# withterm/term

Measured on NVIDIA B200. Metric: rows/sec scanned per suite (numeric business-rules suite, 100M rows x 8 cols per GPU), higher is better.
Workload: dtype f64

## Files before the change

term_b200/csrc/capi.cpp:

```cpp
#include <cstring>

#include "engine.hpp"
#include "hashpart.hpp"
#include "radix_sort.cuh"
#include "regex_dfa.hpp"

namespace tg {
const char* last_error_cstr();
Column* table_get_or_add(Table& t, const std::string& name, int32_t dtype);
void table_append_host(Table& t, const std::string& name, int32_t dtype, int64_t n, const void* values,
                       const int32_t* offsets, const uint8_t* validity, int64_t bit_offset);
void table_append_parquet_chunk(Table& t, const std::string& name, int32_t dtype, int32_t max_def_level, int32_t codec,
                                const uint8_t* chunk, int64_t n_bytes, int64_t num_values);
int32_t parquet_inspect_chunk(const uint8_t* chunk, int64_t n_bytes, tg_parquet_page* pages, int32_t cap);
int64_t parquet_chunk_validity(const uint8_t* chunk, int64_t n_bytes, int64_t num_values, uint8_t* out_bits);
int64_t parquet_snappy_decompress(const uint8_t* src, int64_t n, uint8_t* dst, int64_t cap);
int64_t parquet_page_decompress(int32_t codec, const uint8_t* src, int64_t n, uint8_t* dst, int64_t cap);
void table_set_column_arrow_type(Table& t, const std::string& name, const std::string& fmt);
int64_t parquet_decode_to_plain(int32_t encoding, int32_t elem_width, const uint8_t* src, int64_t n, int64_t n_values, uint8_t* dst, int64_t cap);
void table_adopt_device(Table& t, const std::string& name, int32_t dtype, int64_t n, const void* d_values,
                        const int32_t* d_offsets, const uint8_t* d_validity, int64_t n_value_bytes);
void table_append_arrow(Table& t, const void* schema_p, const void* array_p);
}

// ... 52 lines not shown
        cudaError_t ce = cudaGetDeviceCount(&n);
        if (ce != cudaSuccess || n == 0)
            throw Error(TG_ERR_CUDA, std::string("no CUDA device available (termgpu has no CPU fallback): ") +
                                         cudaGetErrorString(ce));
        if (device < 0 || device >= n) throw Error(TG_ERR_INVALID_ARG, "device index out of range");
        TG_CUDA(cudaSetDevice(device));
        auto* h = new tg_engine();
        Engine& e = h->e;
        e.device = device;
        cudaDeviceProp prop{};
        TG_CUDA(cudaGetDeviceProperties(&prop, device));
        e.sm_count = prop.multiProcessorCount;
        TG_CUDA(cudaStreamCreateWithFlags(&e.stream, cudaStreamNonBlocking));
        TG_CUDA(cudaStreamCreateWithFlags(&e.copy_stream, cudaStreamNonBlocking));
        for (auto& ev : e.ev) TG_CUDA(cudaEventCreate(&ev));
        e.pinned_bytes = 32u << 20;
        for (int i = 0; i < 2; ++i) {
            TG_CUDA(cudaMallocHost(&e.pinned[i], e.pinned_bytes));
            TG_CUDA(cudaEventCreateWithFlags(&e.pinned_free[i], cudaEventDisableTiming));
        }
        *out = h;
    });
}

void tg_engine_destroy(tg_engine* h) {
    if (!h) return;
    Engine& e = h->e;
    cudaSetDevice(e.device);
    cudaDeviceSynchronize();
    rank_session_destroy(e);
// ... 764 lines not shown
```

term_b200/csrc/engine.cu:

```cuda
#include "engine.hpp"

#include <algorithm>
#include <cmath>
#include <cstdlib>
#include <cstring>
#include <ctime>

namespace tg {

constexpr size_t PINNED_CHUNK = 32u << 20;
constexpr size_t PAD = 256;

static size_t round_up(size_t x, size_t a) { return (x + a - 1) / a * a; }

uint8_t* Engine::scratch(size_t bytes) {
    if (bytes > scratch_cap) {
        TG_CUDA(cudaStreamSynchronize(stream));
        if (d_scratch) TG_CUDA(cudaFree(d_scratch));
        scratch_cap = round_up(std::max(bytes, (size_t)1 << 20), 1 << 20);
        TG_CUDA(cudaMalloc(&d_scratch, scratch_cap));
    }
    return d_scratch;
}

// ... 128 lines not shown
    for (size_t i = 0; i < tc.size(); ++i)
        if (tc[i].col == c) {
            tc[i].need_values |= need_values;
            return (int)i;
        }
    tc.push_back(TileCol{c, need_values});
    return (int)tc.size() - 1;
}

static std::string no_field_msg(const Table& t, const std::string& col) {
    return "Schema error: No field named " + col + ". Valid fields are " + t.valid_fields() + ".";
}

__global__ void scan_states_kernel(const ScanAggOut* __restrict__ out, const ScanOpMeta* __restrict__ metas, int n_ops, DevAggRec* __restrict__ states);

static void run_scan_pass(Engine& e, Table& t, Plan& p, std::vector<ScanOp>& ops) {
    if (ops.empty()) return;
    auto P = std::make_unique<ScanParams>();
    memset(P.get(), 0, sizeof(ScanParams));
    std::vector<TileCol> tcols;
    struct OpCols {
        int c0 = -1, c1 = -1;
    };
    std::vector<OpCols> oc(ops.size());
    for (size_t i = 0; i < ops.size(); ++i) {
        ScanOp& o = ops[i];
        if (o.kind == UNIT_COUNT) oc[i].c0 = tile_col_index(tcols, o.c0, false);
        else if (o.kind == UNIT_NUM_F64 || o.kind == UNIT_NUM_I64) oc[i].c0 = tile_col_index(tcols, o.c0, true);
        else if (o.kind == UNIT_PAIR) {
            oc[i].c0 = tile_col_index(tcols, o.c0, true);
            oc[i].c1 = tile_col_index(tcols, o.c1, true);
        } else if (o.kind == UNIT_PRED || o.kind == UNIT_TERMS) {
            for (size_t k = 0; k < o.pred_cols.size(); ++k) {
                bool need_values = true;
// ... 64 lines not shown
            break;
        }
    }
    if (n_stages < 2) throw Error(TG_ERR_UNSUPPORTED, "scan pass does not fit in shared memory");

    std::vector<uint32_t> val_off(tcols.size(), 0), bit_off(tcols.size(), 0);
    stage_bytes_for(tile_rows, &val_off, &bit_off);
    P->n_rows = t.n_rows;
    P->tile_rows = tile_rows;
    P->n_tiles = (t.n_rows + tile_rows - 1) / tile_rows;
    P->n_cols = (int)tcols.size();
    P->n_stages = n_stages;
    P->stage_bytes = (uint32_t)stage_bytes;
    for (size_t i = 0; i < tcols.size(); ++i) {
        Column* c = tcols[i].col;
        ScanColDesc& d = P->tab.cols[i];
        d.values = tcols[i].need_values ? c->values.p : nullptr;
        d.validity = c->validity.p;
        d.kind = c->dtype == TG_FLOAT64 ? SC_F64 : c->dtype == TG_INT64 ? SC_I64 : c->dtype == TG_BOOL ? SC_BOOL : SC_BITS;
        if (!tcols[i].need_values) d.kind = SC_BITS;
        d.smem_val_off = val_off[i];
        d.smem_bits_off = bit_off[i];
        d.pivot = c->pivot;
        d.ipivot = c->ipivot;
        d.pivot_is_element = c->pivot_set ? 1 : 0;
    }
    int term_off = 0;
    struct UnitTmp {
        ScanUnitDesc d;
        double cost;
    };
    std::vector<UnitTmp> units;
    int code_off = 0;
    for (size_t i = 0; i < ops.size(); ++i) {
        ScanOp& o = ops[i];
        int this_code_off = code_off;
        if (o.kind == UNIT_PRED) {
            for (auto ins : o.code) {
                auto fix = [&](uint8_t kind, uint16_t& idx) {
                    if (kind == PK_COL_F64 || kind == PK_COL_I64 || kind == PK_COL_I64_AS_F64 || kind == PK_COL_BOOL)
                        idx = (uint16_t)tile_col_index(tcols, o.pred_cols[idx], true);
                };
                fix(ins.a_kind, ins.a_idx);
                fix(ins.b_kind, ins.b_idx);
                P->tab.code[code_off++] = ins;
            }
        }
        if (o.kind == UNIT_TERMS) {
            this_code_off = term_off;
            for (auto tm : o.terms) {
                tm.col = tile_col_index(tcols, o.pred_cols[tm.col], false);
                if (term_off >= SCAN_MAX_TERMS) throw Error(TG_ERR_UNSUPPORTED, "too many predicate terms in one scan pass");
                P->tab.terms[term_off++] = tm;
            }
        }
        const int r = reps[i];
        const int chunks = tile_rows / 128;
        for (int k = 0; k < r; ++k) {
            UnitTmp u{};
            u.d.kind = o.kind;
            u.d.c0 = oc[i].c0;
            u.d.c1 = oc[i].c1;
            u.d.row0 = (k * chunks / r) * 128;
            u.d.nrows = ((k + 1) * chunks / r) * 128 - u.d.row0;
            u.d.agg = (int)i;
            u.d.code_off = this_code_off;
            u.d.code_len = o.kind == UNIT_TERMS ? (int)o.terms.size() : (int)o.code.size();
            u.d.c0_is_i64 = o.c0 && o.c0->dtype == TG_INT64;
// ... 3 lines not shown
            units.push_back(u);
        }
    }
    std::vector<int> order(units.size());
    for (size_t i = 0; i < order.size(); ++i) order[i] = (int)i;
    std::stable_sort(order.begin(), order.end(), [&](int a, int b) { return units[a].cost > units[b].cost; });
    double load[SCAN_CONSUMER_WARPS] = {0};
    int owned[SCAN_CONSUMER_WARPS] = {0};
    for (int idx : order) {
        int best = -1;
        for (int w = 0; w < SCAN_CONSUMER_WARPS; ++w)
            if (owned[w] < SCAN_WARP_UNITS && (best < 0 || load[w] < load[best])) best = w;
        if (best < 0) throw Error(TG_ERR_UNSUPPORTED, "too many aggregates in one scan pass");
        units[idx].d.warp = best;
        load[best] += units[idx].cost;
        P->tab.warp_units[best][1 + owned[best]] = idx;
        P->tab.warp_units[best][0] = ++owned[best];
    }
    P->n_units = (int)units.size();
    P->n_state_units = units.size() <= (size_t)SCAN_CONSUMER_WARPS ? 0 : (int)units.size();
    P->n_aggs = (int)ops.size();
    P->n_code = code_off;
    P->n_terms = term_off;
    for (size_t i = 0; i < units.size(); ++i) P->tab.units[i] = units[i].d;

    const int grid = (int)std::min<int64_t>(std::max<int64_t>(P->n_tiles, 1), e.sm_count);
    const size_t partial_bytes = (size_t)grid * P->n_units * SCAN_STATE_SLOTS * 8;
    const size_t out_bytes = ops.size() * sizeof(ScanAggOut);
    uint8_t* scr = e.scratch(round_up(partial_bytes, 256) + out_bytes);
    P->partials = reinterpret_cast<uint64_t*>(scr);
    ScanAggOut* d_out = reinterpret_cast<ScanAggOut*>(scr + round_up(partial_bytes, 256));

    TG_CUDA(cudaEventRecord(e.ev[0], e.stream));
    TG_CUDA(scan_launch(*P, grid, d_out, e.stream));
    TG_CUDA(cudaEventRecord(e.ev[1], e.stream));
    e.launches += 2;
    p.stats.launches += 2;
    if (e.fused) {
        FusedScan& fz = *e.fused;
        ScanOpMeta* hm = fz.h_metas + fz.n_metas;
        for (size_t i = 0; i < ops.size(); ++i) {
            hm[i] = ScanOpMeta{ops[i].kind, ops[i].agg, ops[i].c0 ? ops[i].c0->pivot : 0.0, ops[i].c1 ? ops[i].c1->pivot : 0.0, (uint64_t)t.n_rows};
            fz.from_device[ops[i].agg] = 1;
        }
        scan_states_kernel<<<1, 64, 0, e.stream>>>(d_out, hm, (int)ops.size(), fz.d_states);
        TG_CUDA(cudaGetLastError());
        fz.n_metas += (int)ops.size();
        e.launches += 1;
        p.stats.launches += 1;
        return;
    }
    ScanAggOut* h_out = reinterpret_cast<ScanAggOut*>(e.host_scratch(out_bytes));
    TG_CUDA(cudaMemcpyAsync(h_out, d_out, out_bytes, cudaMemcpyDeviceToHost, e.stream));
    TG_CUDA(cudaStreamSynchronize(e.stream));
    float ms = 0;
    TG_CUDA(cudaEventElapsedTime(&ms, e.ev[0], e.ev[1]));
    p.stats.scan_ms += ms;
    p.stats.gpu_ms += ms;

    auto u2d = [](uint64_t u) {
        double d;
        memcpy(&d, &u, 8);
        return d;
    };
    for (size_t i = 0; i < ops.size(); ++i) {
        Agg& a = p.aggs[ops[i].agg];
        const uint64_t* s = h_out[i].s;
        switch (ops[i].kind) {
            case UNIT_COUNT:
                a.u[0] = (uint64_t)t.n_rows;
                a.u[1] = s[S_N];
                break;
            case UNIT_NUM_F64:
            case UNIT_NUM_I64:
                a.u[0] = s[S_N];
                a.f[0] = ops[i].c0->pivot;
                a.f[1] = u2d(s[S_SD]);
                a.f[2] = u2d(s[S_SDD]);
                a.f[5] = (double)s[S_N] * ops[i].c0->pivot + u2d(s[S_SD]);
                if (ops[i].kind == UNIT_NUM_I64) {
                    a.u[1] = s[S_ISUM];
                    a.u[2] = s[S_MIN];
                    a.u[3] = s[S_MAX];
                    a.u[4] = 1;
                } else {
                    a.f[3] = u2d(s[S_MIN]);
                    a.f[4] = u2d(s[S_MAX]);
                }
                break;
            case UNIT_PAIR:
                a.u[0] = s[P_N];
                a.f[0] = ops[i].c0->pivot;
                a.f[1] = ops[i].c1->pivot;
                a.f[2] = u2d(s[P_SX]);
                a.f[3] = u2d(s[P_SY]);
                a.f[4] = u2d(s[P_SXX]);
                a.f[5] = u2d(s[P_SYY]);
                a.f[6] = u2d(s[P_SXY]);
                break;
            case UNIT_PRED:
            case UNIT_TERMS:
                a.u[0] = s[0];
                a.u[1] = ops[i].kind == UNIT_PRED ? s[1] : 0;
                a.u[2] = (uint64_t)t.n_rows;
                break;
        }
    }
}
// ... 89 lines not shown

__global__ void widen_kernel(const uint32_t* __restrict__ src, uint64_t* __restrict__ dst, int64_t n, int is_float) {
    for (int64_t i = (int64_t)blockIdx.x * blockDim.x + threadIdx.x; i < n; i += (int64_t)gridDim.x * blockDim.x) {
        const uint32_t v = __ldg(src + i);
        dst[i] = is_float ? (uint64_t)__double_as_longlong((double)__uint_as_float(v)) : (uint64_t)(int64_t)(int32_t)v;
    }
}

Column* numeric_view(Engine& e, Column* c) {
    if (!c) return nullptr;
    if (c->dtype == TG_INT64 || c->dtype == TG_FLOAT64) return c;
    if (c->dtype != TG_INT32 && c->dtype != TG_FLOAT32) return nullptr;
    if (!c->wide) c->wide = std::make_unique<Column>();
    Column& w = *c->wide;
    if (w.n_rows != c->n_rows || !w.values.p) {
        e.sync_copies();
        w.name = c->name;
        w.dtype = c->dtype == TG_INT32 ? TG_INT64 : TG_FLOAT64;
        e.dev_reserve(w.values, (size_t)c->n_rows * 8, 0);
        if (c->n_rows > 0) {
            const int grid = (int)std::max<int64_t>(1, std::min<int64_t>((c->n_rows + 255) / 256, (int64_t)e.sm_count * 16));
            widen_kernel<<<grid, 256, 0, e.stream>>>(reinterpret_cast<const uint32_t*>(c->values.p), reinterpret_cast<uint64_t*>(w.values.p),
                                                     c->n_rows, c->dtype == TG_FLOAT32 ? 1 : 0);
            TG_CUDA(cudaGetLastError());
            e.launches += 1;
            const int64_t head = std::min<int64_t>(c->n_rows, 65536);
            std::vector<uint8_t> hv((size_t)head * 8), hb((size_t)(head + 7) / 8);
            TG_CUDA(cudaMemcpyAsync(hv.data(), w.values.p, hv.size(), cudaMemcpyDeviceToHost, e.stream));
            if (c->validity.p) TG_CUDA(cudaMemcpyAsync(hb.data(), c->validity.p, hb.size(), cudaMemcpyDeviceToHost, e.stream));
            TG_CUDA(cudaStreamSynchronize(e.stream));
// ... 510 lines not shown
            }
            if (t.n_rows > 0) {
                str_like_kernel<<<grid, 256, 0, e.stream>>>((const int32_t*)col->offsets.p, col->values.p, t.n_rows, d_tok, d_tok + m, (int32_t)m,
                                                            (uint32_t*)v->values.p);
                launched();
            }
            p.stats.bytes_scanned += (uint64_t)(t.n_rows + 1) * 4 + (uint64_t)col->value_bytes;
            return col_node(v);
        }
    }
    auto copy = std::make_shared<Expr>(*ex);
    for (auto& a : copy->args) a = rewrite_string_compares(a, e, t, p, vc);
    return copy;
}

void exec_scan_jobs(Engine& e, Table& t, Plan& p, const std::vector<int>& agg_ids) {
    VirtualCols virtuals(e);
    std::vector<ScanOp> ops;
    uint64_t bytes = 0;
    std::vector<Column*> counted_vals, counted_bits;
    auto count_bytes = [&](Column* c, bool values) {
        if (values && std::find(counted_vals.begin(), counted_vals.end(), c) == counted_vals.end()) {
            counted_vals.push_back(c);
            bytes += c->dtype == TG_BOOL ? (uint64_t)(t.n_rows + 7) / 8 : (uint64_t)t.n_rows * 8;
        }
        if (c->validity.p && std::find(counted_bits.begin(), counted_bits.end(), c) == counted_bits.end()) {
            counted_bits.push_back(c);
            bytes += (uint64_t)(t.n_rows + 7) / 8;
        }
    };
    std::vector<std::pair<int, int>> valid_from_num;
// ... 16 lines not shown
        ScanOp o;
        o.agg = id;
        auto col = [&](const std::string& name) -> Column* {
            Column* c = t.find(name);
            if (!c) {
                a.err = TG_ERR_COLUMN_NOT_FOUND;
                a.err_msg = no_field_msg(t, name);
            }
            return c;
        };
        auto numeric = [&](Column*& c) {
            if (Column* v = c->temporal ? nullptr : numeric_view(e, c)) {
                if (v != c || c->src_type) {
                    a.narrow = 1 | (c->src_unsigned ? 2 : 0);
                    a.narrow_name = c->src_type ? c->src_type : (c->dtype == TG_INT32 ? "Int32" : "Float32");
                }
                c = v;
                return true;
            }
            a.err = TG_ERR_TYPE_MISMATCH;
            a.err_msg = "Error during planning: numeric aggregate is not supported for column '" + c->name +
                        "' of this type";
            return false;
        };
        switch (a.kind) {
            case A_VALID: {
                Column* c = col(a.cols[0]);
                if (!c) break;
                if (!c->validity.p) {
                    a.u[0] = (uint64_t)t.n_rows;
                    a.u[1] = (uint64_t)t.n_rows;
                    break;
                }
                o.kind = UNIT_COUNT;
                o.c0 = c;
                o.cost = 0.2;
                count_bytes(c, false);
                ops.push_back(std::move(o));
            } break;
            case A_NUM: {
                Column* c = col(a.cols[0]);
                if (!c || !numeric(c)) break;
                o.kind = c->dtype == TG_INT64 ? UNIT_NUM_I64 : UNIT_NUM_F64;
                o.c0 = c;
                o.flags = a.flags ? a.flags : 7;
                if (c->dtype != TG_INT64) o.flags &= ~4;
// ... 41 lines not shown
                        compile_predicate(expr, res, o.code);
                        o.kind = UNIT_PRED;
                        o.cost = 10.0 + 25.0 * (double)o.code.size();
                    }
                } catch (Error& er) {
                    a.err = er.code;
                    a.err_msg = er.msg;
                    break;
                }
                for (auto* c : o.pred_cols) count_bytes(c, true);
                ops.push_back(std::move(o));
            } break;
            default: break;
        }
    }
    p.stats.bytes_scanned += bytes;
    struct FoldFill {
        Plan& p;
        Table& t;
        std::vector<std::pair<int, int>>& v;
        ~FoldFill() {
            if (p_fused) {
                for (auto& pr : v) p_fused->folds.push_back(pr);
                return;
            }
            for (auto& pr : v) {
                p.aggs[pr.first].u[0] = (uint64_t)t.n_rows;
                p.aggs[pr.first].u[1] = p.aggs[pr.second].u[0];
            }
        }
        FusedScan* p_fused;
    } fold_fill{p, t, valid_from_num, e.fused};
    if (t.n_rows == 0) {
        for (auto& o : ops)
            if (p.aggs[o.agg].kind == A_PRED) p.aggs[o.agg].u[2] = 0;
        return;
    }
    auto ordinal = [&](const ScanOp& o) {
        const Column* c = o.c0 ? o.c0 : (o.pred_cols.empty() ? nullptr : o.pred_cols[0]);
        if (!c) return -1;
        for (size_t i = 0; i < t.cols.size(); ++i)
            if (t.cols[i].get() == c || t.cols[i]->wide.get() == c) return (int)i;
        return (int)t.cols.size();
    };
    std::vector<std::pair<int, size_t>> op_key(ops.size());
    for (size_t i = 0; i < ops.size(); ++i) op_key[i] = {ordinal(ops[i]), i};
    std::stable_sort(op_key.begin(), op_key.end(), [](const std::pair<int, size_t>& a, const std::pair<int, size_t>& b) { return a.first < b.first; });
    {
// ... 15 lines not shown
        std::vector<ScanOp> pass;
        int code = 0, terms = 0;
        std::vector<const Column*> cols;
        while (i < ops.size() && pass.size() < (size_t)SCAN_CONSUMER_WARPS) {
            const int add_code = (int)ops[i].code.size();
            const int add_terms = ops[i].kind == UNIT_TERMS ? (int)ops[i].terms.size() : 0;
            std::vector<const Column*> with = cols;
            op_cols(ops[i], with);
            if (!pass.empty() && (code + add_code > SCAN_MAX_CODE || terms + add_terms > SCAN_MAX_TERMS || with.size() > (size_t)SCAN_MAX_COLS)) break;
            code += add_code;
            terms += add_terms;
            cols.swap(with);
            pass.push_back(std::move(ops[i]));
            ++i;
        }
        std::vector<int> pass_aggs;
        for (auto& o : pass) pass_aggs.push_back(o.agg);
        try {
            run_scan_pass(e, t, p, pass);
        } catch (Error& er) {
            if (er.code == TG_ERR_CUDA) throw;
            for (int id : pass_aggs) {
                p.aggs[id].err = er.code;
                p.aggs[id].err_msg = er.msg;
            }
        }
    }
}


void execute_partial(Engine& e, Plan& p, const std::string& table_name) {
    std::lock_guard<std::mutex> g(e.mu);
    TG_CUDA(cudaSetDevice(e.device));
    p.reset_partials();
    p.stats = tg_exec_stats{};
    p.executed = false;
    e.sync_copies();
    auto it = e.tables.find(table_name);
    Table* t = it == e.tables.end() ? nullptr : it->second.get();
    std::vector<int> scan_ids, string_ids, kll_ids, length_ids, grouped_ids;
    for (size_t i = 0; i < p.aggs.size(); ++i) {
        Agg& a = p.aggs[i];
        if (a.err != TG_OK) continue;
// ... 173 lines not shown
```

term_b200/csrc/engine.hpp:

```cpp
#pragma once
#include <cuda_runtime.h>

#include <map>
#include <memory>
#include <mutex>
#include <string>
#include <vector>

#include "common.hpp"
#include "plan.hpp"
#include "scan_defs.h"

namespace tg {

#define TG_CUDA(expr)                                                                                   \
    do {                                                                                                \
        cudaError_t _e = (expr);                                                                        \
        if (_e != cudaSuccess)                                                                          \
            throw ::tg::Error(TG_ERR_CUDA, std::string(#expr) + ": " + cudaGetErrorString(_e));         \
    } while (0)

struct Engine;
struct RankSession;

// ... 21 lines not shown
    bool adopted = false;
    std::unique_ptr<Column> wide;
    const char* src_type = nullptr;
    bool src_unsigned = false;
    bool temporal = false;
    char temporal_unit = 0;
    int elem_bytes() const {
        switch (dtype) {
            case TG_INT64: case TG_FLOAT64: return 8;
            case TG_INT32: case TG_FLOAT32: return 4;
            default: return 0;
        }
    }
};

struct Table {
    Engine* eng = nullptr;
    std::string name;
    std::vector<std::unique_ptr<Column>> cols;
    int64_t n_rows = 0;
    Column* find(const std::string& n) {
        for (auto& c : cols)
            if (c->name == n) return c.get();
        return nullptr;
    }
    std::string valid_fields() const {
        std::string s;
        for (size_t i = 0; i < cols.size(); ++i) {
            if (i) s += ", ";
            s += name + "." + cols[i]->name;
        }
        return s;
    }
};

// ... 122 lines not shown

void mailbox_create(Engine& e, int world, int rank, size_t slot_bytes, void* handle_out );
void mailbox_open(Engine& e, const void* handles );
void mailbox_destroy(Engine& e);
bool mailbox_exchange(Engine& e, const uint8_t* blob, size_t n, std::vector<std::vector<uint8_t>>& out);
void mailbox_exchange_device(Engine& e, size_t payload_bytes, std::vector<std::vector<uint8_t>>& out);

void comm_unique_id(void* id128);
void comm_init(Engine& e, const void* id128, int world, int rank);
void comm_destroy(Engine& e);
int64_t comm_shuffle_column(Engine& e, const std::string& table, const std::string& column, const std::string& shard_name, bool allow_range);
bool comm_rank_exchange(Engine& e, int64_t* n_recv, uint64_t* rank_base, uint64_t* total);
int64_t comm_shuffle_fingerprints(Engine& e, const std::string& table, const std::vector<std::string>& columns, const std::string& shard_name);

size_t scan_smem_bytes(const ScanParams& P);
cudaError_t scan_launch(const ScanParams& P, int grid, ScanAggOut* d_out, cudaStream_t stream);

}
```

term_b200/csrc/scan.cu:

```cuda
#include <cfloat>
#include <cstddef>
#include <cstdio>
#include <math_constants.h>

#include "ptx.cuh"
#include "scan_defs.h"

namespace tg {

extern __shared__ __align__(128) uint8_t scan_smem[];

typedef uint64_t Slots[SCAN_STATE_SLOTS];

__device__ __forceinline__ uint32_t tail_mask(int base_row, int rows_in_tile) {
    const int rem = rows_in_tile - base_row;
    return rem >= 32 ? 0xffffffffu : (rem <= 0 ? 0u : ((1u << rem) - 1u));
}
__device__ __forceinline__ double u2d(uint64_t u) { return __longlong_as_double((long long)u); }
__device__ __forceinline__ uint64_t d2u(double d) { return (uint64_t)__double_as_longlong(d); }

__device__ __forceinline__ uint32_t vword(const ScanColDesc& c, const uint8_t* stage, int word) {
    return c.validity ? reinterpret_cast<const uint32_t*>(stage + c.smem_bits_off)[word] : 0xffffffffu;
}
__device__ __forceinline__ uint32_t word_or_ones(const uint32_t* bits, bool has_bits, int g) { return has_bits ? bits[g] : 0xffffffffu; }
// ... 801 lines not shown
            break;
        case UNIT_TERMS: run_unit<SINGLE, TermsUnit>(p, T, ud, st, lane, stage, rows, partial); break;
        default: run_unit<SINGLE, PredUnit>(p, T, ud, st, lane, stage, rows, partial); break;
    }
}

__global__ void __launch_bounds__(SCAN_THREADS, 1) scan_kernel(const __grid_constant__ ScanParams P) {
    const int warp = threadIdx.x >> 5, lane = threadIdx.x & 31;
    uint8_t* stages = scan_smem;
    uint64_t* state = reinterpret_cast<uint64_t*>(scan_smem + (size_t)P.n_stages * P.stage_bytes);
    uint64_t* full = state + (size_t)P.n_state_units * SCAN_STATE_SLOTS * 32;
    uint64_t* empty = full + P.n_stages;
    ScanTables* T = reinterpret_cast<ScanTables*>(empty + P.n_stages);

    {
        const uint32_t* src = reinterpret_cast<const uint32_t*>(&P.tab);
        uint32_t* dst = reinterpret_cast<uint32_t*>(T);
        auto copy = [&](size_t off, size_t bytes) {
            for (uint32_t i = threadIdx.x; i < bytes / 4; i += blockDim.x) dst[off / 4 + i] = src[off / 4 + i];
        };
        copy(offsetof(ScanTables, cols), sizeof(ScanColDesc) * P.n_cols);
        copy(offsetof(ScanTables, units), sizeof(ScanUnitDesc) * P.n_units);
        copy(offsetof(ScanTables, code), sizeof(PredInstr) * P.n_code);
        copy(offsetof(ScanTables, terms), sizeof(ScanTerm) * P.n_terms);
        copy(offsetof(ScanTables, warp_units), sizeof(T->warp_units));
    }
    if (threadIdx.x == 0) {
        for (int s = 0; s < P.n_stages; ++s) {
            mbar_init(&full[s], 1);
            mbar_init(&empty[s], SCAN_CONSUMER_WARPS);
        }
// ... 81 lines not shown
            }
            __syncwarp();
            for (int k = 0; k < n_mine; ++k) {
                const int u = T->warp_units[cw][1 + k];
                const uint64_t* st = state + (size_t)u * SCAN_STATE_SLOTS * 32;
                Slots r;
#pragma unroll
                for (int sl = 0; sl < SCAN_STATE_SLOTS; ++sl) r[sl] = st[sl * 32 + lane];
                reduce_store(T->units[u].kind, r, P.partials + ((size_t)blockIdx.x * P.n_units + u) * SCAN_STATE_SLOTS, lane);
            }
        }
    }
}

constexpr int FIN_THREADS = 128;
__global__ void __launch_bounds__(FIN_THREADS) scan_finalize_kernel(const __grid_constant__ ScanParams P, int n_ctas, ScanAggOut* out) {
    const int agg = blockIdx.x, tid = threadIdx.x, lane = tid & 31, warp = tid >> 5;
    __shared__ int ulist[SCAN_MAX_UNITS];
    __shared__ int s_nu, s_kind;
    __shared__ uint64_t red[FIN_THREADS / 32][SCAN_STATE_SLOTS];
    if (tid == 0) {
        int nu = 0, kind = -1;
        for (int u = 0; u < P.n_units; ++u)
            if (P.tab.units[u].agg == agg) {
                ulist[nu++] = u;
                kind = P.tab.units[u].kind;
            }
        s_nu = nu;
        s_kind = kind;
    }
    __syncthreads();
    const int nu = s_nu, kind = s_kind;
    if (kind < 0) return;
    uint64_t acc[SCAN_STATE_SLOTS];
    int op[SCAN_STATE_SLOTS];
#pragma unroll
    for (int k = 0; k < SCAN_STATE_SLOTS; ++k) {
        op[k] = slot_op(kind, k);
        acc[k] = slot_identity(kind, k);
    }
    const int total = n_ctas * nu;
    for (int i = tid; i < total; i += FIN_THREADS) {
        const int b = i / nu, u = ulist[i - b * nu];
        const ulonglong2* rec = reinterpret_cast<const ulonglong2*>(P.partials + ((size_t)b * P.n_units + u) * SCAN_STATE_SLOTS);
#pragma unroll
        for (int k = 0; k < SCAN_STATE_SLOTS / 2; ++k) {
            const ulonglong2 v = rec[k];
            acc[2 * k] = slot_combine(op[2 * k], acc[2 * k], v.x);
            acc[2 * k + 1] = slot_combine(op[2 * k + 1], acc[2 * k + 1], v.y);
        }
    }
#pragma unroll
    for (int k = 0; k < SCAN_STATE_SLOTS; ++k) {
#pragma unroll
        for (int m = 16; m > 0; m >>= 1) acc[k] = slot_combine(op[k], acc[k], shfl_xor_u64(acc[k], m));
        if (lane == 0) red[warp][k] = acc[k];
    }
    __syncthreads();
    if (tid < SCAN_STATE_SLOTS) {
        uint64_t v = red[0][tid];
        const int o = slot_op(kind, tid);
        for (int w = 1; w < FIN_THREADS / 32; ++w) v = slot_combine(o, v, red[w][tid]);
        out[agg].s[tid] = v;
    }
}

size_t scan_smem_bytes(const ScanParams& P) {
    return (size_t)P.n_stages * P.stage_bytes + (size_t)P.n_state_units * SCAN_STATE_SLOTS * 32 * 8 +
           (size_t)2 * P.n_stages * 8 + sizeof(ScanTables);
}

cudaError_t scan_launch(const ScanParams& P, int grid, ScanAggOut* d_out, cudaStream_t stream) {
    size_t smem = scan_smem_bytes(P);
    cudaError_t e = cudaFuncSetAttribute(scan_kernel, cudaFuncAttributeMaxDynamicSharedMemorySize, 227 * 1024);
    if (e != cudaSuccess) return e;
    scan_kernel<<<grid, SCAN_THREADS, smem, stream>>>(P);
    e = cudaGetLastError();
    if (e != cudaSuccess) return e;
    scan_finalize_kernel<<<P.n_aggs, FIN_THREADS, 0, stream>>>(P, grid, d_out);
    return cudaGetLastError();
}

}
```

term_b200/csrc/scan_defs.h:

```cpp
#pragma once
#include <stdint.h>

namespace tg {

constexpr int SCAN_MAX_COLS = 32;
constexpr int SCAN_MAX_UNITS = 48;
constexpr int SCAN_MAX_CODE = 128;
constexpr int SCAN_MAX_TERMS = 32;
constexpr int SCAN_UNIT_TERMS = 4;
#ifndef TG_SCAN_CONSUMER_WARPS
#define TG_SCAN_CONSUMER_WARPS 16
#endif
constexpr int SCAN_CONSUMER_WARPS = TG_SCAN_CONSUMER_WARPS;
constexpr int SCAN_THREADS = (SCAN_CONSUMER_WARPS + 1) * 32;
constexpr int SCAN_STATE_SLOTS = 8;
constexpr int SCAN_MAX_STAGES = 8;
constexpr int SCAN_WARP_UNITS = 7;

enum : int32_t { SC_F64 = 0, SC_I64 = 1, SC_BITS = 2 , SC_BOOL = 3  };

struct ScanColDesc {
    const uint8_t* values;
    const uint8_t* validity;
    int32_t kind;
// ... 82 lines not shown
    int32_t col;
    int32_t kind;
    int32_t cmp_mask;
    int32_t pad;
    uint64_t imm;
};

struct ScanTables {
    ScanColDesc cols[SCAN_MAX_COLS];
    ScanUnitDesc units[SCAN_MAX_UNITS];
    PredInstr code[SCAN_MAX_CODE];
    ScanTerm terms[SCAN_MAX_TERMS];
    int32_t warp_units[SCAN_CONSUMER_WARPS][SCAN_WARP_UNITS + 1];
};

struct ScanParams {
    int64_t n_rows;
    int64_t n_tiles;
    int32_t tile_rows;
    int32_t n_cols;
    int32_t n_units;
    int32_t n_stages;
    uint32_t stage_bytes;
    int32_t n_aggs;
    int32_t n_code;
    int32_t n_terms;
    int32_t n_state_units;
    uint64_t* partials;
    ScanTables tab;
};

struct ScanAggOut {
    uint64_t s[SCAN_STATE_SLOTS];
};

}
```

term_b200/csrc/tables.cu:

```cuda
#include <algorithm>
#include <cstring>

#include "engine.hpp"

namespace tg {

static size_t round_up(size_t x, size_t a) { return (x + a - 1) / a * a; }

void set_pivot_host(Column& c, int32_t dtype, int64_t n, const void* values, const uint8_t* validity,
                    int64_t bit_offset) {
    if (c.pivot_set || (dtype != TG_INT64 && dtype != TG_FLOAT64)) return;
    double cand[5];
    int64_t icand[5];
    int m = 0;
    for (int64_t i = 0; i < n && i < 65536 && m < 5; ++i) {
        bool ok = !validity || ((validity[(bit_offset + i) >> 3] >> ((bit_offset + i) & 7)) & 1);
        if (!ok) continue;
        if (dtype == TG_INT64) {
            icand[m] = reinterpret_cast<const int64_t*>(values)[i];
            cand[m] = (double)icand[m];
            ++m;
        } else {
            double v = reinterpret_cast<const double*>(values)[i];
            if (v == v && v - v == 0.0) {
// ... 37 lines not shown
    } else {
        for (int64_t i = 0; i < n; ++i) {
            const int64_t s = src_off + i;
            const int bit = (src[s >> 3] >> (s & 7)) & 1;
            const int64_t o = shift + i;
            tmp[o >> 3] |= (uint8_t)(bit << (o & 7));
            z += !bit;
        }
    }
    if (zeros) *zeros = z;
    tail = (total & 7) ? tmp[out_bytes - 1] : 0;
    e.h2d(buf.p + first_byte, tmp.data(), out_bytes);
}

Column* table_get_or_add(Table& t, const std::string& name, int32_t dtype) {
    Column* c = t.find(name);
    if (c) {
        if (c->dtype != dtype) throw Error(TG_ERR_TYPE_MISMATCH, "column '" + name + "' was registered with a different type");
        return c;
    }
    validate_identifier(name);
    auto nc = std::make_unique<Column>();
    nc->name = name;
    nc->dtype = dtype;
    t.cols.push_back(std::move(nc));
    return t.cols.back().get();
}

void append_validity(Engine& e, Column& c, int64_t have, const uint8_t* validity, int64_t bit_offset, int64_t n) {
    bool has_nulls = false;
// ... 174 lines not shown
        f.dtype = TG_INT64, f.temporal = true, f.src_type = "Timestamp", f.temporal_unit = fmt[2];
    else if (fmt == "tDs" || fmt == "tDm" || fmt == "tDu" || fmt == "tDn") f.dtype = TG_INT64, f.temporal = true, f.src_type = "Duration";
    else throw Error(TG_ERR_UNSUPPORTED, std::string("Arrow format '") + fmt + "' of column '" + column + "' is not supported");
    return f;
}

void table_set_column_arrow_type(Table& t, const std::string& name, const std::string& fmt) {
    Engine& e = *t.eng;
    std::lock_guard<std::mutex> g(e.mu);
    Column* c = t.find(name);
    if (!c) throw Error(TG_ERR_COLUMN_NOT_FOUND, "Schema error: No field named " + name + ". Valid fields are " + t.valid_fields() + ".");
    const ArrowFormat f = arrow_format(fmt, name.c_str());
    if (f.dtype != c->dtype || f.large_offsets) throw Error(TG_ERR_TYPE_MISMATCH, "column '" + name + "' does not store Arrow format '" + fmt + "'");
    if (f.src_w == 4 || f.src_w == 8)
        throw Error(TG_ERR_UNSUPPORTED, "column '" + name + "': Arrow format '" + fmt + "' cannot be declared on stored values");
    c->src_type = f.src_type;
    c->src_unsigned = f.src_unsigned;
    c->temporal = f.temporal;
    c->temporal_unit = f.temporal_unit;
}

void table_append_arrow(Table& t, const void* schema_p, const void* array_p) {
    const ArrowSchema* sc = (const ArrowSchema*)schema_p;
    const ArrowArray* ar = (const ArrowArray*)array_p;
    if (!sc || !ar || !sc->format || strcmp(sc->format, "+s") != 0)
        throw Error(TG_ERR_INVALID_ARG, "expected a struct-typed ArrowArray (a RecordBatch)");
    if (ar->offset != 0) throw Error(TG_ERR_UNSUPPORTED, "sliced struct arrays are not supported");
    for (int64_t i = 0; i < sc->n_children; ++i) {
        const ArrowSchema* cs = sc->children[i];
        const ArrowArray* ca = ar->children[i];
// ... 72 lines not shown
```

Measured before the change: 191.5 billion.

## Cache compiled scan passes per table and move scan tables to device memory

Compiles each scan pass once into a cached entry keyed by aggregate definitions and env knobs. Per-pass tables, including a new precomputed finalize unit list, are uploaded once to a persistent device block, so the large ScanTables struct no longer travels as a kernel parameter. The smem opt-in attribute is set once at engine creation, and the finalize kernel batches its partial loads. The cache adds invalidation complexity: it must be cleared when columns change, and a stale entry would give wrong results.

New measurement: 195.2 billion, median of 6. 2.0% higher.

```diff
diff --git a/term_b200/csrc/capi.cpp b/term_b200/csrc/capi.cpp
--- a/term_b200/csrc/capi.cpp
+++ b/term_b200/csrc/capi.cpp
@@ -90,6 +90,7 @@
         TG_CUDA(cudaStreamCreateWithFlags(&e.stream, cudaStreamNonBlocking));
         TG_CUDA(cudaStreamCreateWithFlags(&e.copy_stream, cudaStreamNonBlocking));
         for (auto& ev : e.ev) TG_CUDA(cudaEventCreate(&ev));
+        TG_CUDA(scan_opt_in());
         e.pinned_bytes = 32u << 20;
         for (int i = 0; i < 2; ++i) {
             TG_CUDA(cudaMallocHost(&e.pinned[i], e.pinned_bytes));
diff --git a/term_b200/csrc/engine.cu b/term_b200/csrc/engine.cu
--- a/term_b200/csrc/engine.cu
+++ b/term_b200/csrc/engine.cu
@@ -166,10 +166,12 @@
 
 __global__ void scan_states_kernel(const ScanAggOut* __restrict__ out, const ScanOpMeta* __restrict__ metas, int n_ops, DevAggRec* __restrict__ states);
 
-static void run_scan_pass(Engine& e, Table& t, Plan& p, std::vector<ScanOp>& ops) {
-    if (ops.empty()) return;
-    auto P = std::make_unique<ScanParams>();
-    memset(P.get(), 0, sizeof(ScanParams));
+static CompiledPass compile_scan_pass(Engine& e, Table& t, std::vector<ScanOp>& ops) {
+    CompiledPass cp;
+    cp.host = std::make_unique<ScanPassTables>();
+    memset(cp.host.get(), 0, sizeof(ScanPassTables));
+    ScanParams* P = &cp.P;
+    ScanTables& tab = cp.host->tab;
     std::vector<TileCol> tcols;
     struct OpCols {
         int c0 = -1, c1 = -1;
@@ -264,7 +266,7 @@
     P->stage_bytes = (uint32_t)stage_bytes;
     for (size_t i = 0; i < tcols.size(); ++i) {
         Column* c = tcols[i].col;
-        ScanColDesc& d = P->tab.cols[i];
+        ScanColDesc& d = tab.cols[i];
         d.values = tcols[i].need_values ? c->values.p : nullptr;
         d.validity = c->validity.p;
         d.kind = c->dtype == TG_FLOAT64 ? SC_F64 : c->dtype == TG_INT64 ? SC_I64 : c->dtype == TG_BOOL ? SC_BOOL : SC_BITS;
@@ -293,7 +295,7 @@
                 };
                 fix(ins.a_kind, ins.a_idx);
                 fix(ins.b_kind, ins.b_idx);
-                P->tab.code[code_off++] = ins;
+                tab.code[code_off++] = ins;
             }
         }
         if (o.kind == UNIT_TERMS) {
@@ -301,7 +303,7 @@
             for (auto tm : o.terms) {
                 tm.col = tile_col_index(tcols, o.pred_cols[tm.col], false);
                 if (term_off >= SCAN_MAX_TERMS) throw Error(TG_ERR_UNSUPPORTED, "too many predicate terms in one scan pass");
-                P->tab.terms[term_off++] = tm;
+                tab.terms[term_off++] = tm;
             }
         }
         const int r = reps[i];
@@ -335,25 +337,45 @@
         if (best < 0) throw Error(TG_ERR_UNSUPPORTED, "too many aggregates in one scan pass");
         units[idx].d.warp = best;
         load[best] += units[idx].cost;
-        P->tab.warp_units[best][1 + owned[best]] = idx;
-        P->tab.warp_units[best][0] = ++owned[best];
+        tab.warp_units[best][1 + owned[best]] = idx;
+        tab.warp_units[best][0] = ++owned[best];
     }
     P->n_units = (int)units.size();
     P->n_state_units = units.size() <= (size_t)SCAN_CONSUMER_WARPS ? 0 : (int)units.size();
     P->n_aggs = (int)ops.size();
     P->n_code = code_off;
     P->n_terms = term_off;
-    for (size_t i = 0; i < units.size(); ++i) P->tab.units[i] = units[i].d;
-
-    const int grid = (int)std::min<int64_t>(std::max<int64_t>(P->n_tiles, 1), e.sm_count);
-    const size_t partial_bytes = (size_t)grid * P->n_units * SCAN_STATE_SLOTS * 8;
-    const size_t out_bytes = ops.size() * sizeof(ScanAggOut);
-    uint8_t* scr = e.scratch(round_up(partial_bytes, 256) + out_bytes);
-    P->partials = reinterpret_cast<uint64_t*>(scr);
-    ScanAggOut* d_out = reinterpret_cast<ScanAggOut*>(scr + round_up(partial_bytes, 256));
-
+    for (size_t i = 0; i < units.size(); ++i) tab.units[i] = units[i].d;
+    ScanFinalize& fin = cp.host->fin;
+    for (size_t a = 0; a < ops.size(); ++a) {
+        fin.off[a + 1] = fin.off[a];
+        for (size_t u = 0; u < units.size(); ++u)
+            if (units[u].d.agg == (int)a) {
+                fin.units[fin.off[a + 1]++] = (int)u;
+                fin.kind[a] = units[u].d.kind;
+            }
+    }
+    cp.grid = (int)std::min<int64_t>(std::max<int64_t>(P->n_tiles, 1), e.sm_count);
+    for (auto& o : ops) cp.ops.push_back(ScanPassOp{o.kind, o.agg, o.c0 ? o.c0->pivot : 0.0, o.c1 ? o.c1->pivot : 0.0});
+    return cp;
+}
+
+static size_t pass_device_bytes(const CompiledPass& cp) {
+    return round_up(cp.partial_bytes(), 256) + round_up(cp.ops.size() * sizeof(ScanAggOut), 256) + round_up(sizeof(ScanPassTables), 256);
+}
+static void place_pass(Engine& e, CompiledPass& cp, uint8_t* d) {
+    cp.P.partials = reinterpret_cast<uint64_t*>(d);
+    d += round_up(cp.partial_bytes(), 256);
+    cp.d_out = reinterpret_cast<ScanAggOut*>(d);
+    d += round_up(cp.ops.size() * sizeof(ScanAggOut), 256);
+    cp.P.tables = reinterpret_cast<const ScanPassTables*>(d);
+    TG_CUDA(cudaMemcpyAsync(d, cp.host.get(), sizeof(ScanPassTables), cudaMemcpyHostToDevice, e.stream));
+}
+
+static void run_scan_pass(Engine& e, Table& t, Plan& p, const CompiledPass& cp) {
+    const std::vector<ScanPassOp>& ops = cp.ops;
     TG_CUDA(cudaEventRecord(e.ev[0], e.stream));
-    TG_CUDA(scan_launch(*P, grid, d_out, e.stream));
+    TG_CUDA(scan_launch(cp.P, cp.grid, cp.d_out, e.stream));
     TG_CUDA(cudaEventRecord(e.ev[1], e.stream));
     e.launches += 2;
     p.stats.launches += 2;
@@ -361,18 +383,18 @@
         FusedScan& fz = *e.fused;
         ScanOpMeta* hm = fz.h_metas + fz.n_metas;
         for (size_t i = 0; i < ops.size(); ++i) {
-            hm[i] = ScanOpMeta{ops[i].kind, ops[i].agg, ops[i].c0 ? ops[i].c0->pivot : 0.0, ops[i].c1 ? ops[i].c1->pivot : 0.0, (uint64_t)t.n_rows};
+            hm[i] = ScanOpMeta{ops[i].kind, ops[i].agg, ops[i].pivot0, ops[i].pivot1, (uint64_t)t.n_rows};
             fz.from_device[ops[i].agg] = 1;
         }
-        scan_states_kernel<<<1, 64, 0, e.stream>>>(d_out, hm, (int)ops.size(), fz.d_states);
+        scan_states_kernel<<<1, 64, 0, e.stream>>>(cp.d_out, hm, (int)ops.size(), fz.d_states);
         TG_CUDA(cudaGetLastError());
         fz.n_metas += (int)ops.size();
         e.launches += 1;
         p.stats.launches += 1;
         return;
     }
-    ScanAggOut* h_out = reinterpret_cast<ScanAggOut*>(e.host_scratch(out_bytes));
-    TG_CUDA(cudaMemcpyAsync(h_out, d_out, out_bytes, cudaMemcpyDeviceToHost, e.stream));
+    const ScanAggOut* h_out = cp.h_out;
+    TG_CUDA(cudaMemcpyAsync(cp.h_out, cp.d_out, ops.size() * sizeof(ScanAggOut), cudaMemcpyDeviceToHost, e.stream));
     TG_CUDA(cudaStreamSynchronize(e.stream));
     float ms = 0;
     TG_CUDA(cudaEventElapsedTime(&ms, e.ev[0], e.ev[1]));
@@ -395,10 +417,10 @@
             case UNIT_NUM_F64:
             case UNIT_NUM_I64:
                 a.u[0] = s[S_N];
-                a.f[0] = ops[i].c0->pivot;
+                a.f[0] = ops[i].pivot0;
                 a.f[1] = u2d(s[S_SD]);
                 a.f[2] = u2d(s[S_SDD]);
-                a.f[5] = (double)s[S_N] * ops[i].c0->pivot + u2d(s[S_SD]);
+                a.f[5] = (double)s[S_N] * ops[i].pivot0 + u2d(s[S_SD]);
                 if (ops[i].kind == UNIT_NUM_I64) {
                     a.u[1] = s[S_ISUM];
                     a.u[2] = s[S_MIN];
@@ -411,8 +433,8 @@
                 break;
             case UNIT_PAIR:
                 a.u[0] = s[P_N];
-                a.f[0] = ops[i].c0->pivot;
-                a.f[1] = ops[i].c1->pivot;
+                a.f[0] = ops[i].pivot0;
+                a.f[1] = ops[i].pivot1;
                 a.f[2] = u2d(s[P_SX]);
                 a.f[3] = u2d(s[P_SY]);
                 a.f[4] = u2d(s[P_SXX]);
@@ -532,6 +554,9 @@
     if (!c->wide) c->wide = std::make_unique<Column>();
     Column& w = *c->wide;
     if (w.n_rows != c->n_rows || !w.values.p) {
+        for (auto& kv : e.tables)
+            for (auto& tc : kv.second->cols)
+                if (tc.get() == c) kv.second->clear_scan_cache();
         e.sync_copies();
         w.name = c->name;
         w.dtype = c->dtype == TG_INT32 ? TG_INT64 : TG_FLOAT64;
@@ -1072,7 +1097,59 @@
     return copy;
 }
 
+ScanCacheEntry::~ScanCacheEntry() {
+    if (d_block) eng->dev_free(d_block, d_bytes);
+    if (h_block) cudaFreeHost(h_block);
+}
+
+constexpr size_t SCAN_CACHE_ENTRIES = 8;
+
+static std::string scan_cache_key(const Plan& p, const std::vector<int>& agg_ids) {
+    std::string k;
+    for (const char* knob : {"TG_SCAN_TILE_ROWS", "TG_SCAN_MIN_STAGES", "TG_SCAN_UNITS"}) {
+        const char* v = getenv(knob);
+        k += v ? v : "";
+        k += '\x1e';
+    }
+    for (int id : agg_ids) {
+        const Agg& a = p.aggs[id];
+        k += std::to_string(id) + '\x1f' + std::to_string((int)a.kind) + '\x1f' + std::to_string(a.flags) + '\x1f' + a.key + '\x1e';
+    }
+    return k;
+}
+
+static void run_cached_scan(Engine& e, Table& t, Plan& p, const ScanCacheEntry& ce) {
+    p.stats.bytes_scanned += ce.bytes_scanned;
+    for (size_t i = 0; i < ce.narrow.size(); ++i) {
+        p.aggs[ce.narrow[i].first].narrow = ce.narrow[i].second;
+        p.aggs[ce.narrow[i].first].narrow_name = ce.narrow_name[i];
+    }
+    for (int id : ce.all_rows) {
+        p.aggs[id].u[0] = (uint64_t)t.n_rows;
+        p.aggs[id].u[1] = (uint64_t)t.n_rows;
+    }
+    for (const CompiledPass& cp : ce.passes) run_scan_pass(e, t, p, cp);
+    for (auto& pr : ce.folds) {
+        if (e.fused) {
+            e.fused->folds.push_back(pr);
+        } else {
+            p.aggs[pr.first].u[0] = (uint64_t)t.n_rows;
+            p.aggs[pr.first].u[1] = p.aggs[pr.second].u[0];
+        }
+    }
+}
+
 void exec_scan_jobs(Engine& e, Table& t, Plan& p, const std::vector<int>& agg_ids) {
+    const std::string key = scan_cache_key(p, agg_ids);
+    for (size_t i = 0; i < t.scan_cache.size(); ++i)
+        if (t.scan_cache[i]->key == key) {
+            std::rotate(t.scan_cache.begin() + i, t.scan_cache.begin() + i + 1, t.scan_cache.end());
+            run_cached_scan(e, t, p, *t.scan_cache.back());
+            return;
+        }
+    auto ce = std::make_unique<ScanCacheEntry>();
+    ce->eng = &e;
+    ce->key = key;
     VirtualCols virtuals(e);
     std::vector<ScanOp> ops;
     uint64_t bytes = 0;
@@ -1119,6 +1196,8 @@
                 if (v != c || c->src_type) {
                     a.narrow = 1 | (c->src_unsigned ? 2 : 0);
                     a.narrow_name = c->src_type ? c->src_type : (c->dtype == TG_INT32 ? "Int32" : "Float32");
+                    ce->narrow.emplace_back(id, a.narrow);
+                    ce->narrow_name.push_back(a.narrow_name);
                 }
                 c = v;
                 return true;
@@ -1133,8 +1212,7 @@
                 Column* c = col(a.cols[0]);
                 if (!c) break;
                 if (!c->validity.p) {
-                    a.u[0] = (uint64_t)t.n_rows;
-                    a.u[1] = (uint64_t)t.n_rows;
+                    ce->all_rows.push_back(id);
                     break;
                 }
                 o.kind = UNIT_COUNT;
@@ -1206,7 +1284,6 @@
             default: break;
         }
     }
-    p.stats.bytes_scanned += bytes;
     struct FoldFill {
         Plan& p;
         Table& t;
@@ -1223,7 +1300,12 @@
         }
         FusedScan* p_fused;
     } fold_fill{p, t, valid_from_num, e.fused};
+    for (int id : ce->all_rows) {
+        p.aggs[id].u[0] = (uint64_t)t.n_rows;
+        p.aggs[id].u[1] = (uint64_t)t.n_rows;
+    }
     if (t.n_rows == 0) {
+        p.stats.bytes_scanned += bytes;
         for (auto& o : ops)
             if (p.aggs[o.agg].kind == A_PRED) p.aggs[o.agg].u[2] = 0;
         return;
@@ -1269,19 +1351,54 @@
             pass.push_back(std::move(ops[i]));
             ++i;
         }
-        std::vector<int> pass_aggs;
-        for (auto& o : pass) pass_aggs.push_back(o.agg);
         try {
-            run_scan_pass(e, t, p, pass);
+            ce->passes.push_back(compile_scan_pass(e, t, pass));
         } catch (Error& er) {
             if (er.code == TG_ERR_CUDA) throw;
-            for (int id : pass_aggs) {
-                p.aggs[id].err = er.code;
-                p.aggs[id].err_msg = er.msg;
-            }
-        }
-    }
-}
+            for (auto& o : pass) {
+                p.aggs[o.agg].err = er.code;
+                p.aggs[o.agg].err_msg = er.msg;
+            }
+        }
+    }
+    bool cacheable = virtuals.cols.empty();
+    for (int id : agg_ids) cacheable &= p.aggs[id].err == TG_OK;
+    if (!cacheable) {
+        p.stats.bytes_scanned += bytes;
+        for (CompiledPass& cp : ce->passes) {
+            const size_t out_bytes = cp.ops.size() * sizeof(ScanAggOut);
+            place_pass(e, cp, e.scratch(pass_device_bytes(cp)));
+            cp.h_out = reinterpret_cast<ScanAggOut*>(e.host_scratch(out_bytes));
+            run_scan_pass(e, t, p, cp);
+        }
+        return;
+    }
+    ce->folds = valid_from_num;
+    ce->bytes_scanned = bytes;
+    fold_fill.v.clear();
+    size_t d_bytes = 0, h_bytes = 0;
+    for (const CompiledPass& cp : ce->passes) {
+        d_bytes += pass_device_bytes(cp);
+        h_bytes += round_up(cp.ops.size() * sizeof(ScanAggOut), 64);
+    }
+    if (d_bytes) {
+        ce->d_block = e.dev_alloc(d_bytes);
+        ce->d_bytes = d_bytes;
+        TG_CUDA(cudaMallocHost(&ce->h_block, h_bytes));
+    }
+    uint8_t* d = ce->d_block;
+    uint8_t* h = ce->h_block;
+    for (CompiledPass& cp : ce->passes) {
+        place_pass(e, cp, d);
+        cp.h_out = reinterpret_cast<ScanAggOut*>(h);
+        d += pass_device_bytes(cp);
+        h += round_up(cp.ops.size() * sizeof(ScanAggOut), 64);
+    }
+    if (t.scan_cache.size() >= SCAN_CACHE_ENTRIES) t.scan_cache.erase(t.scan_cache.begin());
+    t.scan_cache.push_back(std::move(ce));
+    run_cached_scan(e, t, p, *t.scan_cache.back());
+}
+
 
 
 void execute_partial(Engine& e, Plan& p, const std::string& table_name) {
diff --git a/term_b200/csrc/engine.hpp b/term_b200/csrc/engine.hpp
--- a/term_b200/csrc/engine.hpp
+++ b/term_b200/csrc/engine.hpp
@@ -59,11 +59,42 @@
     }
 };
 
+struct ScanPassOp {
+    int32_t kind, agg;
+    double pivot0, pivot1;
+};
+struct CompiledPass {
+    ScanParams P{};
+    int grid = 0;
+    std::unique_ptr<ScanPassTables> host;
+    std::vector<ScanPassOp> ops;
+    ScanAggOut* d_out = nullptr;
+    ScanAggOut* h_out = nullptr;
+    size_t partial_bytes() const { return (size_t)grid * P.n_units * SCAN_STATE_SLOTS * 8; }
+};
+
+struct ScanCacheEntry {
+    Engine* eng = nullptr;
+    std::string key;
+    std::vector<CompiledPass> passes;
+    uint64_t bytes_scanned = 0;
+    std::vector<int> all_rows;
+    std::vector<std::pair<int, int>> folds;
+    std::vector<std::pair<int, int32_t>> narrow;
+    std::vector<const char*> narrow_name;
+    uint8_t* d_block = nullptr;
+    size_t d_bytes = 0;
+    uint8_t* h_block = nullptr;
+    ~ScanCacheEntry();
+};
+
 struct Table {
     Engine* eng = nullptr;
     std::string name;
     std::vector<std::unique_ptr<Column>> cols;
     int64_t n_rows = 0;
+    std::vector<std::unique_ptr<ScanCacheEntry>> scan_cache;
+    void clear_scan_cache() { scan_cache.clear(); }
     Column* find(const std::string& n) {
         for (auto& c : cols)
             if (c->name == n) return c.get();
@@ -216,6 +247,7 @@
 int64_t comm_shuffle_fingerprints(Engine& e, const std::string& table, const std::vector<std::string>& columns, const std::string& shard_name);
 
 size_t scan_smem_bytes(const ScanParams& P);
+cudaError_t scan_opt_in();
 cudaError_t scan_launch(const ScanParams& P, int grid, ScanAggOut* d_out, cudaStream_t stream);
 
 }
diff --git a/term_b200/csrc/scan.cu b/term_b200/csrc/scan.cu
--- a/term_b200/csrc/scan.cu
+++ b/term_b200/csrc/scan.cu
@@ -839,7 +839,7 @@
     ScanTables* T = reinterpret_cast<ScanTables*>(empty + P.n_stages);
 
     {
-        const uint32_t* src = reinterpret_cast<const uint32_t*>(&P.tab);
+        const uint32_t* src = reinterpret_cast<const uint32_t*>(&P.tables->tab);
         uint32_t* dst = reinterpret_cast<uint32_t*>(T);
         auto copy = [&](size_t off, size_t bytes) {
             for (uint32_t i = threadIdx.x; i < bytes / 4; i += blockDim.x) dst[off / 4 + i] = src[off / 4 + i];
@@ -951,24 +951,15 @@
 }
 
 constexpr int FIN_THREADS = 128;
-__global__ void __launch_bounds__(FIN_THREADS) scan_finalize_kernel(const __grid_constant__ ScanParams P, int n_ctas, ScanAggOut* out) {
+__global__ void __launch_bounds__(FIN_THREADS) scan_finalize_kernel(const ScanParams P, int n_ctas, ScanAggOut* out) {
     const int agg = blockIdx.x, tid = threadIdx.x, lane = tid & 31, warp = tid >> 5;
     __shared__ int ulist[SCAN_MAX_UNITS];
-    __shared__ int s_nu, s_kind;
     __shared__ uint64_t red[FIN_THREADS / 32][SCAN_STATE_SLOTS];
-    if (tid == 0) {
-        int nu = 0, kind = -1;
-        for (int u = 0; u < P.n_units; ++u)
-            if (P.tab.units[u].agg == agg) {
-                ulist[nu++] = u;
-                kind = P.tab.units[u].kind;
-            }
-        s_nu = nu;
-        s_kind = kind;
-    }
+    const ScanFinalize& F = P.tables->fin;
+    const int u0 = F.off[agg], nu = F.off[agg + 1] - u0, kind = F.kind[agg];
+    if (tid < nu) ulist[tid] = F.units[u0 + tid];
     __syncthreads();
-    const int nu = s_nu, kind = s_kind;
-    if (kind < 0) return;
+    if (nu == 0) return;
     uint64_t acc[SCAN_STATE_SLOTS];
     int op[SCAN_STATE_SLOTS];
 #pragma unroll
@@ -977,14 +968,27 @@
         acc[k] = slot_identity(kind, k);
     }
     const int total = n_ctas * nu;
-    for (int i = tid; i < total; i += FIN_THREADS) {
-        const int b = i / nu, u = ulist[i - b * nu];
-        const ulonglong2* rec = reinterpret_cast<const ulonglong2*>(P.partials + ((size_t)b * P.n_units + u) * SCAN_STATE_SLOTS);
-#pragma unroll
-        for (int k = 0; k < SCAN_STATE_SLOTS / 2; ++k) {
-            const ulonglong2 v = rec[k];
-            acc[2 * k] = slot_combine(op[2 * k], acc[2 * k], v.x);
-            acc[2 * k + 1] = slot_combine(op[2 * k + 1], acc[2 * k + 1], v.y);
+    constexpr int FIN_BATCH = 8;
+    for (int i0 = tid; i0 < total; i0 += FIN_THREADS * FIN_BATCH) {
+        ulonglong2 v[FIN_BATCH][SCAN_STATE_SLOTS / 2];
+#pragma unroll
+        for (int j = 0; j < FIN_BATCH; ++j) {
+            const int i = i0 + j * FIN_THREADS;
+            if (i < total) {
+                const int b = i / nu, u = ulist[i - b * nu];
+                const ulonglong2* rec = reinterpret_cast<const ulonglong2*>(P.partials + ((size_t)b * P.n_units + u) * SCAN_STATE_SLOTS);
+#pragma unroll
+                for (int k = 0; k < SCAN_STATE_SLOTS / 2; ++k) v[j][k] = rec[k];
+            }
+        }
+#pragma unroll
+        for (int j = 0; j < FIN_BATCH; ++j) {
+            if (i0 + j * FIN_THREADS >= total) break;
+#pragma unroll
+            for (int k = 0; k < SCAN_STATE_SLOTS / 2; ++k) {
+                acc[2 * k] = slot_combine(op[2 * k], acc[2 * k], v[j][k].x);
+                acc[2 * k + 1] = slot_combine(op[2 * k + 1], acc[2 * k + 1], v[j][k].y);
+            }
         }
     }
 #pragma unroll
@@ -1007,12 +1011,13 @@
            (size_t)2 * P.n_stages * 8 + sizeof(ScanTables);
 }
 
+cudaError_t scan_opt_in() {
+    return cudaFuncSetAttribute(scan_kernel, cudaFuncAttributeMaxDynamicSharedMemorySize, 227 * 1024);
+}
+
 cudaError_t scan_launch(const ScanParams& P, int grid, ScanAggOut* d_out, cudaStream_t stream) {
-    size_t smem = scan_smem_bytes(P);
-    cudaError_t e = cudaFuncSetAttribute(scan_kernel, cudaFuncAttributeMaxDynamicSharedMemorySize, 227 * 1024);
-    if (e != cudaSuccess) return e;
-    scan_kernel<<<grid, SCAN_THREADS, smem, stream>>>(P);
-    e = cudaGetLastError();
+    scan_kernel<<<grid, SCAN_THREADS, scan_smem_bytes(P), stream>>>(P);
+    cudaError_t e = cudaGetLastError();
     if (e != cudaSuccess) return e;
     scan_finalize_kernel<<<P.n_aggs, FIN_THREADS, 0, stream>>>(P, grid, d_out);
     return cudaGetLastError();
diff --git a/term_b200/csrc/scan_defs.h b/term_b200/csrc/scan_defs.h
--- a/term_b200/csrc/scan_defs.h
+++ b/term_b200/csrc/scan_defs.h
@@ -120,6 +120,17 @@
     int32_t warp_units[SCAN_CONSUMER_WARPS][SCAN_WARP_UNITS + 1];
 };
 
+struct ScanFinalize {
+    int32_t off[SCAN_MAX_UNITS + 1];
+    int32_t units[SCAN_MAX_UNITS];
+    int32_t kind[SCAN_MAX_UNITS];
+};
+
+struct ScanPassTables {
+    ScanTables tab;
+    ScanFinalize fin;
+};
+
 struct ScanParams {
     int64_t n_rows;
     int64_t n_tiles;
@@ -133,7 +144,7 @@
     int32_t n_terms;
     int32_t n_state_units;
     uint64_t* partials;
-    ScanTables tab;
+    const ScanPassTables* tables;
 };
 
 struct ScanAggOut {
diff --git a/term_b200/csrc/tables.cu b/term_b200/csrc/tables.cu
--- a/term_b200/csrc/tables.cu
+++ b/term_b200/csrc/tables.cu
@@ -75,6 +75,7 @@
 }
 
 Column* table_get_or_add(Table& t, const std::string& name, int32_t dtype) {
+    t.clear_scan_cache();
     Column* c = t.find(name);
     if (c) {
         if (c->dtype != dtype) throw Error(TG_ERR_TYPE_MISMATCH, "column '" + name + "' was registered with a different type");
@@ -279,6 +280,7 @@
     if (f.dtype != c->dtype || f.large_offsets) throw Error(TG_ERR_TYPE_MISMATCH, "column '" + name + "' does not store Arrow format '" + fmt + "'");
     if (f.src_w == 4 || f.src_w == 8)
         throw Error(TG_ERR_UNSUPPORTED, "column '" + name + "': Arrow format '" + fmt + "' cannot be declared on stored values");
+    t.clear_scan_cache();
     c->src_type = f.src_type;
     c->src_unsigned = f.src_unsigned;
     c->temporal = f.temporal;
```
